# Banksylel/Restrictive-Hierarchical-Semantic-Segmentation

Measured on AMD Instinct MI355X. Metric: train images/sec (620x620, hier-HRNet-W48), higher is better.
Workload: dtype f32 (fp16x2 split on fp16 MFMA, 22-bit operands, fp32 accumulate; exact-fp32 MFMA on the small problems); 1 GPU; HRNet-W48 hierarchical (class_tree_tl.json), 620x620, batch 4 per GPU, train_epoch batch body (fwd L passes, prediction prep + metrics, CE+Dice+consistency, bwd, grad all-reduce, AdamW, metric vectors, one D2H readback of loss+metrics); global_batch=4, parallelism=dp1, launch=launch tape replay, rccl_ranks=1, level_passes=batched (one launch per layer for all L passes)

## Files before the change

restrictive-hierarchical-semantic-segmentation_amd/csrc/bn.hip:

```cpp
#include "elem_common.h"
#include "sp_arith.h"

__device__ __forceinline__ void reduce_chunks16(const double* __restrict__ partial, int nchunks, int C, int c,
                                               double& s0, double& s1, double* red) {
  const int lane = threadIdx.x >> 4;
  double a = 0.0, b = 0.0;
  if (c < C) {
    int k = lane;
    for (; k + 48 < nchunks; k += 64) {
      double t0[4], t1[4];
#pragma unroll
      for (int u = 0; u < 4; ++u) {
        t0[u] = partial[((size_t)(k + 16 * u) * 2 + 0) * C + c];
        t1[u] = partial[((size_t)(k + 16 * u) * 2 + 1) * C + c];
      }
#pragma unroll
      for (int u = 0; u < 4; ++u) {
        a += t0[u];
        b += t1[u];
      }
    }
    for (; k < nchunks; k += 16) {
      a += partial[((size_t)k * 2 + 0) * C + c];
      b += partial[((size_t)k * 2 + 1) * C + c];
    }
  }
  red[threadIdx.x * 2] = a;
  red[threadIdx.x * 2 + 1] = b;
  __syncthreads();
  s0 = 0.0;
  s1 = 0.0;
  if (threadIdx.x < 16)
    for (int l = 0; l < 16; ++l) {
      s0 += red[(l * 16 + threadIdx.x) * 2];
      s1 += red[(l * 16 + threadIdx.x) * 2 + 1];
    }
}

__global__ __launch_bounds__(256) void bn_fold_kernel(const float* __restrict__ w, const float* __restrict__ bias,
                                                      const float* __restrict__ gamma, const float* __restrict__ beta,
                                                      const float* __restrict__ rmean, const float* __restrict__ rvar, float eps,
                                                      int row, float* __restrict__ w_out, float* __restrict__ b_out) {
  const int co = blockIdx.x;
  const float s = (gamma ? gamma[co] : 1.f) / sqrtf(rvar[co] + eps);
  for (int i = threadIdx.x; i < row; i += 256) w_out[(size_t)co * row + i] = w[(size_t)co * row + i] * s;
  if (threadIdx.x == 0) b_out[co] = ((bias ? bias[co] : 0.f) - rmean[co]) * s + (beta ? beta[co] : 0.f);
}

#define BN_MAXG 8
struct BnGroupHdr { int n; int blk_end[BN_MAXG]; };
__device__ __forceinline__ int bn_find(const BnGroupHdr& h, int& local, int& nblk) {
  int g = 0;
  while (g + 1 < h.n && (int)blockIdx.x >= h.blk_end[g]) ++g;
  const int lo = g ? h.blk_end[g - 1] : 0;
  local = blockIdx.x - lo;
  nblk = h.blk_end[g] - lo;
  return g;
}
struct BnFwdG { BnGroupHdr h; hrseg_bn_fwd_t p[BN_MAXG]; };
struct BnBwdG { BnGroupHdr h; hrseg_bn_bwd_t p[BN_MAXG]; };

template <bool MASK>
__device__ __forceinline__ void stats_body(const float* __restrict__ a0, int ld0, const float* __restrict__ zmask,
                                           int ldz, int relu, const float* __restrict__ yy, int ldy,
                                           const float* __restrict__ coef, long npix, int C,
                                           double* __restrict__ partial, int chunk, int nchunks, bool bwd,
                                           double* red, int nseg = 1, const unsigned char* __restrict__ bmask = nullptr) {
  const Lanes L = make_lanes(C);
  const int cps = nchunks / nseg, seg = chunk / cps;
  const long seg_pix = npix / nseg;
  const long per = (seg_pix + cps - 1) / cps;
  const long lo = seg * seg_pix + (long)(chunk - seg * cps) * per;
  const long seg_end = (seg + 1) * seg_pix;
  const long hi = (lo + per < seg_end) ? lo + per : seg_end;
  f32x4 s = {0.f, 0.f, 0.f, 0.f}, s2 = {0.f, 0.f, 0.f, 0.f};
  if (L.active) {
    f32x4 mean = {0.f, 0.f, 0.f, 0.f}, rstd = {1.f, 1.f, 1.f, 1.f}, sc = mean, sh = mean;
    if (bwd) {
      mean = ld4(coef + 4 * L.cq);
      rstd = ld4(coef + C + 4 * L.cq);
      sc = ld4(coef + 2 * C + 4 * L.cq);
      sh = ld4(coef + 3 * C + 4 * L.cq);
// ... 303 lines not shown
          a_dg = f32x4{0.f, 0.f, 0.f, 0.f};
          a_db = f32x4{0.f, 0.f, 0.f, 0.f};
          ++b;
          bnd += hw;
          if (gb) {
            gam = ld4(gb + (size_t)b * 2 * C + 4 * L.cq);
            bet = ld4(gb + (size_t)b * 2 * C + C + 4 * L.cq);
          }
        }
        const f32x4 zc = bn_affine(yv[u], sc, sh);
        f32x4 fv;
#pragma unroll
        for (int j = 0; j < 4; ++j) fv[j] = fmaxf(zc[j], 0.f);
        const f32x4 fm = fv * gam + bet;
        f32x4 uu = {0.f, 0.f, 0.f, 0.f};
#pragma unroll
        for (int c = 0; c < CO; ++c) {
          uu += wq[c] * g[u][c];
          a_dw[c] += fm * g[u][c];
          if (L.cq == 0) a_bias[c] += g[u][c];
        }
        a_dg += fv * uu;
        a_db += uu;
        f32x4 gv = gam * uu;
#pragma unroll
        for (int j = 0; j < 4; ++j) gv[j] = zc[j] > 0.f ? gv[j] : 0.f;
        const f32x4 xh = (yv[u] - mean) * rstd;
        s += gv;
        s2 += gv * xh;
      }
    }
    flush_dgb();
  }
#pragma unroll
  for (int j = 0; j < 4; ++j) {
    red[threadIdx.x * 8 + j] = s[j];
    red[threadIdx.x * 8 + 4 + j] = s2[j];
  }
  __syncthreads();
  for (int c = threadIdx.x; c < C; c += 256) {
    double sa = 0.0, sb = 0.0;
    for (int pl = 0; pl < L.P; ++pl) {
      const int t = pl * L.Q + (c >> 2);
      sa += red[t * 8 + (c & 3)];
      sb += red[t * 8 + 4 + (c & 3)];
    }
    a.partial[((size_t)chunk * 2 + 0) * C + c] = sa;
    a.partial[((size_t)chunk * 2 + 1) * C + c] = sb;
  }
  float* fred = reinterpret_cast<float*>(red);
  float* dw = a.dw[seg];
  float* dbias = a.dbias[seg];
  auto reduce_add = [&](float v, float* dst) {
    __syncthreads();
    fred[threadIdx.x] = v;
    __syncthreads();
    if (L.active && L.pl == 0) {
      float t = 0.f;
      for (int q = 0; q < L.P; ++q) t += fred[q * L.Q + L.cq];
      atomicAdd(dst, t);
    }
  };
#pragma unroll
  for (int j = 0; j < 4; ++j)
#pragma unroll
    for (int c = 0; c < CO; ++c)
      if (c < Cout) reduce_add(a_dw[c][j], dw + c * C + 4 * (L.active ? L.cq : 0) + j);
  if (dbias) {
#pragma unroll
    for (int c = 0; c < CO; ++c)
      if (c < Cout) {
        __syncthreads();
        fred[threadIdx.x] = (L.active && L.cq == 0) ? a_bias[c] : 0.f;
        __syncthreads();
        if (threadIdx.x == 0) {
          float t = 0.f;
          for (int q = 0; q < L.P; ++q) t += fred[q * L.Q];
          atomicAdd(dbias + c, t);
        }
      }
  }
}

template <int CO>
__global__ __launch_bounds__(256) void head_bn_bwd_apply_kernel(hrseg_head_bn_t a) {
  const int C = a.F;
  const Lanes L = make_lanes(C);
  float amax = 0.f;
  if (L.active) {
    const double* totals = a.partial + (size_t)a.nchunks * 2 * C;
    const f32x4 mean = ld4(a.coef + 4 * L.cq), rstd = ld4(a.coef + C + 4 * L.cq), scale = ld4(a.coef + 2 * C + 4 * L.cq);
    const f32x4 shift = ld4(a.coef + 3 * C + 4 * L.cq);
    const long hw = a.hw, seg_pix = (long)a.B * hw;
    const float inv = (float)(1.0 / (double)seg_pix);
    for (int seg = 0; seg < a.nseg; ++seg) {
      f32x4 mg, mgx;
#pragma unroll
      for (int j = 0; j < 4; ++j) {
        mg[j] = (float)(totals[(size_t)seg * 2 * C + 4 * L.cq + j]) * inv;
        mgx[j] = (float)(totals[(size_t)seg * 2 * C + C + 4 * L.cq + j]) * inv;
      }
      const float* __restrict__ gb = a.gb[seg];
      const float* __restrict__ w = a.w[seg];
      const float* __restrict__ dzl = a.dzl[seg];
      const int lddz = a.lddzl[seg], Cout = a.Cout[seg];
      f32x4 wq[CO];
#pragma unroll
      for (int c = 0; c < CO; ++c) wq[c] = (c < Cout) ? ld4(w + c * C + 4 * L.cq) : f32x4{0.f, 0.f, 0.f, 0.f};
      for (int b = 0; b < a.B; ++b) {
        const f32x4 gam = gb ? ld4(gb + (size_t)b * 2 * C + 4 * L.cq) : f32x4{1.f, 1.f, 1.f, 1.f};
        const long r0 = (long)b * hw, r1 = r0 + hw;
        for (long r = r0 + (long)blockIdx.x * L.P + L.pl; r < r1; r += (long)gridDim.x * L.P) {
          const long pix = seg * seg_pix + r;
          const f32x4 yv = ld4(a.y + pix * a.ldy + 4 * L.cq);
          f32x4 uu = {0.f, 0.f, 0.f, 0.f};
#pragma unroll
          for (int c = 0; c < CO; ++c) uu += wq[c] * ((c < Cout) ? dzl[r * lddz + c] : 0.f);
          f32x4 gg = gam * uu;
          const f32x4 zz = bn_affine(yv, scale, shift);
#pragma unroll
          for (int j = 0; j < 4; ++j) gg[j] = zz[j] > 0.f ? gg[j] : 0.f;
          const f32x4 xh = (yv - mean) * rstd;
          const f32x4 dyv = scale * (gg - mg - xh * mgx);
          st4(a.dy + pix * a.lddy + 4 * L.cq, dyv);
#pragma unroll
          for (int j = 0; j < 4; ++j) amax = fmaxf(amax, fabsf(dyv[j]));
        }
      }
    }
  }
  if (a.dy_absmax) {
    __shared__ float wmax[4];
#pragma unroll
    for (int o = 32; o > 0; o >>= 1) amax = fmaxf(amax, __shfl_xor(amax, o, 64));
    if ((threadIdx.x & 63) == 0) wmax[threadIdx.x >> 6] = amax;
    __syncthreads();
    if (threadIdx.x == 0) {
      const float m = fmaxf(fmaxf(wmax[0], wmax[1]), fmaxf(wmax[2], wmax[3]));
      if (m > 0.f) atomicMax(reinterpret_cast<unsigned*>(a.dy_absmax) + (blockIdx.x & 63), __float_as_uint(m));
    }
  }
}

extern "C" int hrseg_bn_fold(const float* w, const float* bias, const float* gamma, const float* beta, const float* running_mean,
                             const float* running_var, float eps, int Cout, int row, float* w_out, float* b_out,
                             hrseg_stream_t stream) {
  HRSEG_CHECK_ARG(w && running_mean && running_var && w_out && b_out && Cout > 0 && row > 0, "hrseg_bn_fold: bad arguments");
  hipLaunchKernelGGL(bn_fold_kernel, dim3(Cout), dim3(256), 0, (hipStream_t)stream, w, bias, gamma, beta, running_mean,
                     running_var, eps, row, w_out, b_out);
  HRSEG_LAUNCH_CHECK("bn_fold");
  return 0;
}

static int check_bn_fwd(const hrseg_bn_fwd_t& p, int training, int phases) {
  if (int e = check_c(p.C, "hrseg_bn_fwd_group")) return e;
  const bool stats = training && (phases & 1), finalize = phases & 2, apply = phases & 4;
  HRSEG_CHECK_ARG(p.coef, "hrseg_bn_fwd_group: bad tensor arguments (coef)");
  HRSEG_CHECK_ARG(!(stats || apply) || (p.y && p.ldy >= p.C && p.ldy % 4 == 0), "hrseg_bn_fwd_group: bad tensor arguments (y, ldy)");
  HRSEG_CHECK_ARG(!(stats || apply || (training && finalize)) || p.npix > 0, "hrseg_bn_fwd_group: bad tensor arguments (npix)");
  HRSEG_CHECK_ARG(!apply || (p.z && p.ldz >= p.C && p.ldz % 4 == 0), "hrseg_bn_fwd_group: bad tensor arguments (the apply phase needs z, ldz)");
  HRSEG_CHECK_ARG(!(stats || (training && finalize)) || (p.partial && p.nchunks > 0), "hrseg_bn_fwd_group: training needs partial/nchunks");
  HRSEG_CHECK_ARG(training || !finalize || (p.running_mean && p.running_var), "hrseg_bn_fwd_group: eval needs running stats");
  return 0;
}

extern "C" int hrseg_bn_fwd_group(int n, const hrseg_bn_fwd_t* probs, int training, hrseg_stream_t stream) {
// ... 26 lines not shown
  } else if (phases & 2) {
    for (int i = 0; i < n; ++i) { end += ceil_div(probs[i].C, 64); g.h.blk_end[i] = end; }
    hipLaunchKernelGGL(bn_eval_coef_group_kernel, dim3(end), dim3(64), 0, st, g);
    HRSEG_LAUNCH_CHECK("bn_eval_coef_group");
  }
  if (phases & 4) {
    end = 0;
    for (int i = 0; i < n; ++i) { end += elem_grid(probs[i].npix, probs[i].C); g.h.blk_end[i] = end; }
    hipLaunchKernelGGL(bn_apply_group_kernel, dim3(end), dim3(256), 0, st, g);
    HRSEG_LAUNCH_CHECK("bn_apply_group");
  }
  return 0;
}

extern "C" int hrseg_bn_bwd_group(int n, const hrseg_bn_bwd_t* probs, int eval_mode, hrseg_stream_t stream) {
  return hrseg_bn_bwd_group_phases(n, probs, eval_mode, 7, stream);
}

extern "C" int hrseg_bn_bwd_group_phases(int n, const hrseg_bn_bwd_t* probs, int eval_mode, int phases, hrseg_stream_t stream) {
  HRSEG_CHECK_ARG(n >= 1 && n <= BN_MAXG && probs, "hrseg_bn_bwd_group: n must be 1..%d", BN_MAXG);
  HRSEG_CHECK_ARG(phases > 0 && phases <= 7, "hrseg_bn_bwd_group_phases: phases is a mask of bits 0..2");
  hipStream_t st = (hipStream_t)stream;
  BnBwdG g;
  g.h.n = n;
  for (int i = 0; i < n; ++i) {
    const hrseg_bn_bwd_t& p = probs[i];
    if (int e = check_c(p.C, "hrseg_bn_bwd_group")) return e;
    HRSEG_CHECK_ARG(p.dz && p.y && p.coef && p.dy && p.partial && p.npix > 0 && p.nchunks > 0,
                    "hrseg_bn_bwd_group: bad arguments");
    HRSEG_CHECK_ARG(p.nseg <= 1 || (p.nchunks % p.nseg == 0 && p.npix % p.nseg == 0),
                    "hrseg_bn_bwd_group: nseg=%d must divide nchunks=%d and npix", p.nseg, p.nchunks);
    g.p[i] = p;
  }
  int end = 0;
  bool masked = false;
  for (int i = 0; i < n; ++i) masked = masked || (probs[i].relu && probs[i].relu_mask);
  if (phases & 1) {
    for (int i = 0; i < n; ++i) { end += probs[i].nchunks; g.h.blk_end[i] = end; }
    if (masked) hipLaunchKernelGGL(bn_bwd_reduce_group_kernel<true>, dim3(end), dim3(256), 0, st, g);
    else hipLaunchKernelGGL(bn_bwd_reduce_group_kernel<false>, dim3(end), dim3(256), 0, st, g);
    HRSEG_LAUNCH_CHECK("bn_bwd_reduce_group");
  }
  if (phases & 2) {
    end = 0;
    for (int i = 0; i < n; ++i) { end += ceil_div(probs[i].C, 16); g.h.blk_end[i] = end; }
    hipLaunchKernelGGL(bn_bwd_finalize_group_kernel, dim3(end), dim3(256), 0, st, g);
    HRSEG_LAUNCH_CHECK("bn_bwd_finalize_group");
  }
  if (phases & 4) {
    end = 0;
    for (int i = 0; i < n; ++i) { end += elem_grid(probs[i].npix, probs[i].C); g.h.blk_end[i] = end; }
    hipLaunchKernelGGL(bn_bwd_apply_group_kernel, dim3(end), dim3(256), 0, st, g, eval_mode);
    HRSEG_LAUNCH_CHECK("bn_bwd_apply_group");
  }
  return 0;
}

static int check_head_bn(const hrseg_head_bn_t* p, const char* who, int seg0, int nsegs) {
  HRSEG_CHECK_ARG(p, "%s: NULL problem", who);
  if (int e = check_c(p->F, who)) return e;
  HRSEG_CHECK_ARG(p->y && p->coef && p->partial && p->B > 0 && p->hw > 0 && p->nseg >= 1 && p->nseg <= HRSEG_HEAD_BN_MAX_SEG &&
                      p->nchunks > 0 && p->nchunks % p->nseg == 0 && p->ldy >= p->F && p->ldy % 4 == 0,
                  "%s: bad arguments (F=%d nseg=%d nchunks=%d ldy=%d)", who, p->F, p->nseg, p->nchunks, p->ldy);
  HRSEG_CHECK_ARG(seg0 >= 0 && nsegs >= 1 && seg0 + nsegs <= p->nseg, "%s: segments [%d, %d) of %d", who, seg0, seg0 + nsegs, p->nseg);
  for (int s = seg0; s < seg0 + nsegs; ++s) {
    HRSEG_CHECK_ARG(p->w[s] && p->dzl[s] && p->Cout[s] > 0 && p->Cout[s] <= 8 && p->lddzl[s] >= p->Cout[s],
                    "%s: segment %d: bad head (Cout=%d lddzl=%d)", who, s, p->Cout[s], p->lddzl[s]);
  }
  return 0;
}

extern "C" int hrseg_head_bn_bwd_reduce(const hrseg_head_bn_t* p, int seg0, int nsegs, hrseg_stream_t stream) {
  if (int e = check_head_bn(p, "hrseg_head_bn_bwd_reduce", seg0, nsegs)) return e;
  if (hrseg_g_deterministic) {
    hrseg_set_error("hrseg_head_bn_bwd_reduce: not offered in deterministic mode (atomic sums); use hrseg_head_bwd + hrseg_bn_bwd_group");
    return HRSEG_ERR_UNSUPPORTED;
  }
  int comax = 0;
  for (int s = seg0; s < seg0 + nsegs; ++s) {
    HRSEG_CHECK_ARG(p->dw[s] && (p->gb[s] == nullptr) == (p->dgb[s] == nullptr), "hrseg_head_bn_bwd_reduce: segment %d: dw is required, dgb goes with gb", s);
    comax = p->Cout[s] > comax ? p->Cout[s] : comax;
  }
  const int cps = p->nchunks / p->nseg;
  if (comax <= 4) hipLaunchKernelGGL(head_bn_bwd_reduce_kernel<4>, dim3(nsegs * cps), dim3(256), 0, (hipStream_t)stream, *p, seg0 * cps);
  else hipLaunchKernelGGL(head_bn_bwd_reduce_kernel<8>, dim3(nsegs * cps), dim3(256), 0, (hipStream_t)stream, *p, seg0 * cps);
  HRSEG_LAUNCH_CHECK("head_bn_bwd_reduce");
  return 0;
}

extern "C" int hrseg_head_bn_bwd_apply(const hrseg_head_bn_t* p, hrseg_stream_t stream) {
  if (int e = check_head_bn(p, "hrseg_head_bn_bwd_apply", 0, p ? p->nseg : 1)) return e;
  HRSEG_CHECK_ARG(p->dy && p->lddy >= p->F && p->lddy % 4 == 0, "hrseg_head_bn_bwd_apply: bad dy (lddy=%d)", p->lddy);
  int comax = 0;
  for (int s = 0; s < p->nseg; ++s) comax = p->Cout[s] > comax ? p->Cout[s] : comax;
  const long npix = (long)p->nseg * p->B * p->hw;
  const int grid = elem_grid(npix, p->F);
  if (comax <= 4) hipLaunchKernelGGL(head_bn_bwd_apply_kernel<4>, dim3(grid), dim3(256), 0, (hipStream_t)stream, *p);
  else hipLaunchKernelGGL(head_bn_bwd_apply_kernel<8>, dim3(grid), dim3(256), 0, (hipStream_t)stream, *p);
  HRSEG_LAUNCH_CHECK("head_bn_bwd_apply");
  return 0;
}
```

restrictive-hierarchical-semantic-segmentation_amd/csrc/head_loss.hip:

```cpp
#include "common.h"

#define MAXC 16

struct Groups {
  int n;
  int parent[MAXC];
  int size[MAXC];
};

static int fill_groups(Groups& g, int ngroups, const int* parent, const int* size, int C, int Cprev, const char* who) {
  HRSEG_CHECK_ARG(ngroups >= 0 && ngroups <= MAXC && (ngroups == 0 || (parent && size)), "%s: bad group table", who);
  g.n = ngroups;
  int tot = 0;
  for (int i = 0; i < ngroups; ++i) {
    HRSEG_CHECK_ARG(parent[i] >= 0 && parent[i] < Cprev && size[i] > 0, "%s: group %d out of range", who, i);
    g.parent[i] = parent[i];
    g.size[i] = size[i];
    tot += size[i];
  }
  HRSEG_CHECK_ARG(tot == C || ngroups == 0, "%s: group sizes sum to %d, level has %d channels", who, tot, C);
  return 0;
}

__global__ __launch_bounds__(256) void gap_partial_kernel(const float* __restrict__ p, double* __restrict__ part,
// ... 240 lines not shown
        for (int c = 0; c < CO; ++c) g[i][c] = (c < Cout) ? dz[r * lddz + c] : 0.f;
      }
#pragma unroll
      for (int i = 0; i < U; ++i) one(fv[i], g[i], dold[i], (size_t)b * hw + pix + (long)i * P);
    }
    for (; pix < hi; pix += P) {
      const size_t r = (size_t)b * hw + pix;
      float g[CO];
#pragma unroll
      for (int c = 0; c < CO; ++c) g[c] = (c < Cout) ? dz[r * lddz + c] : 0.f;
      one(*reinterpret_cast<const f32x4*>(f + r * ldf + 4 * cq), g, racc ? *reinterpret_cast<const f32x4*>(df + r * lddf + 4 * cq) : zero, r);
    }
  }
  auto reduce_add = [&](float v, float* dst) {
    red[threadIdx.x] = v;
    __syncthreads();
    if (active && pl == 0) {
      float s = 0.f;
      for (int q = 0; q < P; ++q) s += red[q * Q + cq];
      atomicAdd(dst, s);
    }
    __syncthreads();
  };
#pragma unroll
  for (int j = 0; j < 4; ++j) {
#pragma unroll
    for (int c = 0; c < CO; ++c)
      if (c < Cout) reduce_add(a_dw[c][j], dw + c * F + 4 * cq + j);
    if (dgb) {
      reduce_add(a_dg[j], dgb + (size_t)b * 2 * F + 4 * cq + j);
      reduce_add(a_db[j], dgb + (size_t)b * 2 * F + F + 4 * cq + j);
    }
  }
  if (dbias) {
#pragma unroll
    for (int c = 0; c < CO; ++c)
      if (c < Cout) {
        red[threadIdx.x] = (active && cq == 0) ? a_bias[c] : 0.f;
        __syncthreads();
        if (threadIdx.x == 0) {
          float s = 0.f;
          for (int q = 0; q < P; ++q) s += red[q * Q];
          atomicAdd(dbias + c, s);
        }
        __syncthreads();
      }
  }
}

__device__ __forceinline__ void src_index_ac(int o, float scale, int in_size, int align, int& i0, int& i1, float& l0,
                                             float& l1) {
  float r;
  if (align) {
    r = scale * (float)o;
  } else {
    r = scale * ((float)o + 0.5f) - 0.5f;
    if (r < 0.f) r = 0.f;
  }
  i0 = (int)r;
  if (i0 > in_size - 1) i0 = in_size - 1;
  i1 = i0 + ((i0 < in_size - 1) ? 1 : 0);
  l1 = r - (float)i0;
  l0 = 1.f - l1;
}
__global__ void logits_up_fwd_kernel(const float* __restrict__ in, int ldin, int B, int Hi, int Wi, int C,
                                     float* __restrict__ out, int Ho, int Wo, float sh, float sw, int align) {
  const long i = (long)blockIdx.x * blockDim.x + threadIdx.x;
  const long hw = (long)Ho * Wo;
  if (i >= B * hw) return;
  const int b = (int)(i / hw);
  const long p = i - b * hw;
  const int oy = (int)(p / Wo), ox = (int)(p - (long)oy * Wo);
  int y0, y1, x0, x1;
  float ly0, ly1, lx0, lx1;
  src_index_ac(oy, sh, Hi, align, y0, y1, ly0, ly1);
  src_index_ac(ox, sw, Wi, align, x0, x1, lx0, lx1);
  const float* base = in + (size_t)b * Hi * Wi * ldin;
  for (int c = 0; c < C; ++c) {
    const float v00 = base[((size_t)y0 * Wi + x0) * ldin + c], v01 = base[((size_t)y0 * Wi + x1) * ldin + c];
    const float v10 = base[((size_t)y1 * Wi + x0) * ldin + c], v11 = base[((size_t)y1 * Wi + x1) * ldin + c];
    out[((size_t)b * C + c) * hw + p] = ly0 * (lx0 * v00 + lx1 * v01) + ly1 * (lx0 * v10 + lx1 * v11);
  }
}
__global__ void logits_up_bwd_kernel(const float* __restrict__ dout, int B, int Hi, int Wi, int C,
                                     float* __restrict__ din, int lddin, int Ho, int Wo, float sh, float sw,
                                     int align) {
  const long i = (long)blockIdx.x * blockDim.x + threadIdx.x;
  if (i >= (long)B * Hi * Wi) return;
  const int b = (int)(i / ((long)Hi * Wi));
  const int rem = (int)(i - (long)b * Hi * Wi);
  const int iy = rem / Wi, ix = rem - iy * Wi;
  const long hw = (long)Ho * Wo;
  const float ish = sh > 0.f ? 1.f / sh : 0.f, isw = sw > 0.f ? 1.f / sw : 0.f;
  const float hf = align ? 0.f : 0.5f;
  int oy_lo = 0, oy_hi = Ho - 1, ox_lo = 0, ox_hi = Wo - 1;
  if (sh > 0.f) {
    oy_lo = max(0, (int)floorf(((float)iy - 1.f + hf) * ish - hf) - 1);
    oy_hi = min(Ho - 1, (int)ceilf(((float)iy + 1.f + hf) * ish - hf) + 1);
  }
  if (sw > 0.f) {
    ox_lo = max(0, (int)floorf(((float)ix - 1.f + hf) * isw - hf) - 1);
    ox_hi = min(Wo - 1, (int)ceilf(((float)ix + 1.f + hf) * isw - hf) + 1);
  }
  float s[MAXC];
#pragma unroll
  for (int c = 0; c < MAXC; ++c) s[c] = 0.f;
  for (int oy = oy_lo; oy <= oy_hi; ++oy) {
    int y0, y1;
    float ly0, ly1;
    src_index_ac(oy, sh, Hi, align, y0, y1, ly0, ly1);
    const float wy = (y0 == iy ? ly0 : 0.f) + (y1 == iy ? ly1 : 0.f);
    if (wy == 0.f) continue;
    for (int ox = ox_lo; ox <= ox_hi; ++ox) {
      int x0, x1;
      float lx0, lx1;
      src_index_ac(ox, sw, Wi, align, x0, x1, lx0, lx1);
      const float wx = (x0 == ix ? lx0 : 0.f) + (x1 == ix ? lx1 : 0.f);
      if (wx == 0.f) continue;
      const float wgt = wy * wx;
#pragma unroll
      for (int c = 0; c < MAXC; ++c)
        if (c < C) s[c] = fmaf(wgt, dout[((size_t)b * C + c) * hw + (size_t)oy * Wo + ox], s[c]);
    }
  }
#pragma unroll
  for (int c = 0; c < MAXC; ++c)
    if (c < C) din[i * lddin + c] = s[c];
}

__global__ void sigmoid_fwd_kernel(const float* __restrict__ z, float* __restrict__ p, long n) {
  const long i = (long)blockIdx.x * blockDim.x + threadIdx.x;
  if (i < n) p[i] = 1.f / (1.f + expf(-z[i]));
}
__global__ void sigmoid_bwd_kernel(const float* __restrict__ dp, long sb, long sc, long si,
                                   const float* __restrict__ z, float* __restrict__ dz, int acc, int C, long hw,
                                   long n) {
  const long i = (long)blockIdx.x * blockDim.x + threadIdx.x;
  if (i >= n) return;
  const long bc = i / hw, pix = i - bc * hw;
  const long b = bc / C, c = bc - b * C;
  const float p = 1.f / (1.f + expf(-z[i]));
  const float g = dp[b * sb + c * sc + pix * si] * p * (1.f - p);
  dz[i] = acc ? dz[i] + g : g;
}

#define EPS_GATE 1e-6f
__global__ void compose_fwd_kernel(const float* __restrict__ z, const float* __restrict__ pprev,
                                   float* __restrict__ p, int C, int Cprev, long hw, long n, Groups g) {
  const long i = (long)blockIdx.x * blockDim.x + threadIdx.x;
  if (i >= n) return;
  const long b = i / hw, pix = i - b * hw;
  const float* zb = z + (size_t)b * C * hw + pix;
  float* pb = p + (size_t)b * C * hw + pix;
  int start = 0;
  for (int gi = 0; gi < g.n; ++gi) {
    const int sz = g.size[gi];
    const float pp = pprev[((size_t)b * Cprev + g.parent[gi]) * hw + pix];
    const float lg = logf(pp + EPS_GATE);
    float m = -INFINITY;
    for (int c = 0; c < sz; ++c) m = fmaxf(m, zb[(size_t)(start + c) * hw] + lg);
    float s = 0.f;
    for (int c = 0; c < sz; ++c) s += expf(zb[(size_t)(start + c) * hw] + lg - m);
    const float inv = 1.f / s;
    for (int c = 0; c < sz; ++c) pb[(size_t)(start + c) * hw] = pp * (expf(zb[(size_t)(start + c) * hw] + lg - m) * inv);
    start += sz;
  }
}
__global__ void compose_bwd_kernel(const float* __restrict__ dp, long sb, long sc, long si,
                                   const float* __restrict__ z, const float* __restrict__ pprev,
                                   float* __restrict__ dz, int dz_acc, float* __restrict__ dpprev, int dpp_acc,
                                   int C, int Cprev, long hw, long n, Groups g) {
  const long i = (long)blockIdx.x * blockDim.x + threadIdx.x;
  if (i >= n) return;
  const long b = i / hw, pix = i - b * hw;
  const float* zb = z + (size_t)b * C * hw + pix;
  float dpar[MAXC];
#pragma unroll
  for (int c = 0; c < MAXC; ++c) dpar[c] = 0.f;
  int start = 0;
  for (int gi = 0; gi < g.n; ++gi) {
    const int sz = g.size[gi];
    const float pp = pprev[((size_t)b * Cprev + g.parent[gi]) * hw + pix];
    const float lg = logf(pp + EPS_GATE);
    float m = -INFINITY;
    for (int c = 0; c < sz; ++c) m = fmaxf(m, zb[(size_t)(start + c) * hw] + lg);
    float s = 0.f;
    for (int c = 0; c < sz; ++c) s += expf(zb[(size_t)(start + c) * hw] + lg - m);
    const float inv = 1.f / s;
    float dot = 0.f, dpp = 0.f;
    for (int c = 0; c < sz; ++c) {
      const float q = expf(zb[(size_t)(start + c) * hw] + lg - m) * inv;
      const float d = dp[b * sb + (start + c) * sc + pix * si];
      dot += q * d * pp;
      dpp += d * q;
    }
    float sum_ds = 0.f;
    for (int c = 0; c < sz; ++c) {
      const float q = expf(zb[(size_t)(start + c) * hw] + lg - m) * inv;
      const float d = dp[b * sb + (start + c) * sc + pix * si];
      const float ds = q * (d * pp - dot);
      sum_ds += ds;
      if (dz) {
        float* o = dz + ((size_t)b * C + start + c) * hw + pix;
        *o = dz_acc ? *o + ds : ds;
      }
    }
    dpp += sum_ds / (pp + EPS_GATE);
#pragma unroll
    for (int c = 0; c < MAXC; ++c)
      if (c == g.parent[gi]) dpar[c] += dpp;
// ... 385 lines not shown
  const size_t smem = (size_t)(co * F + co) * sizeof(float);
  const int lp = (F / 4 <= 16) ? 16 : 64;
  long blocks = (hw + (256 / lp) - 1) / (256 / lp);
  const long cap = (2048 + B - 1) / B < 64 ? 64 : (2048 + B - 1) / B;
  if (blocks > cap) blocks = cap;
  dim3 grid((int)blocks, B);
#define HF(LP_, CO_)                                                                                                              \
  do {                                                                                                                            \
    if (coef) hipLaunchKernelGGL((head_fwd_kernel<LP_, CO_, true>), grid, dim3(256), smem, st, f, ldf, coef, gb, w, bias, z, ldz, \
                                 hw, F, Cout);                                                                                    \
    else hipLaunchKernelGGL((head_fwd_kernel<LP_, CO_, false>), grid, dim3(256), smem, st, f, ldf, coef, gb, w, bias, z, ldz, hw, \
                            F, Cout);                                                                                             \
  } while (0)
  if (lp == 16 && co == 4) HF(16, 4);
  else if (lp == 16) HF(16, 8);
  else if (co == 4) HF(64, 4);
  else HF(64, 8);
#undef HF
  HRSEG_LAUNCH_CHECK(who);
  return 0;
}

extern "C" int hrseg_head_fwd(const float* f, int ldf, const float* gb, const float* w, const float* bias, float* z,
                              int ldz, int B, long hw, int F, int Cout, hrseg_stream_t stream) {
  return head_fwd_launch("hrseg_head_fwd", f, ldf, nullptr, gb, w, bias, z, ldz, B, hw, F, Cout, stream);
}

extern "C" int hrseg_head_bn_fwd(const float* y, int ldy, const float* coef, const float* gb, const float* w, const float* bias,
                                 float* z, int ldz, int B, long hw, int F, int Cout, hrseg_stream_t stream) {
  HRSEG_CHECK_ARG(coef, "hrseg_head_bn_fwd: coef is required (hrseg_head_fwd reads a normalised tensor)");
  return head_fwd_launch("hrseg_head_bn_fwd", y, ldy, coef, gb, w, bias, z, ldz, B, hw, F, Cout, stream);
}

extern "C" int hrseg_head_bwd(const float* f, int ldf, const float* gb, const float* w, const float* dz, int lddz,
                              float* df, int lddf, int df_accumulate, float* dw, float* dbias, float* dgb, int B,
                              long hw, int F, int Cout, hrseg_stream_t stream) {
  HRSEG_CHECK_ARG(f && w && dz && dw && B > 0 && hw > 0 && F > 0 && F % 4 == 0 && F <= 1024 && Cout > 0 &&
                      Cout <= 8 && (gb == nullptr) == (dgb == nullptr),
                  "hrseg_head_bwd: bad arguments (F=%d Cout=%d)", F, Cout);
  HRSEG_CHECK_ARG(ldf >= F && ldf % 4 == 0 && lddz >= Cout && (df == nullptr || (lddf >= F && lddf % 4 == 0)),
                  "hrseg_head_bwd: bad row strides (ldf=%d lddz=%d lddf=%d for F=%d Cout=%d)", ldf, lddz, lddf, F, Cout);
  hipStream_t st = (hipStream_t)stream;
  long chunks = 2048 / B;
  if (chunks < 1) chunks = 1;
  long ppb = (hw + chunks - 1) / chunks;
  if (ppb < 64) ppb = 64;
  const int nlaunch = hrseg_g_deterministic ? B : 1;
  if (hrseg_g_deterministic) ppb = hw;
  dim3 grid(ceil_div(hw, ppb), hrseg_g_deterministic ? 1 : B);
  for (int b0 = 0; b0 < nlaunch; ++b0) {
    if (Cout <= 4)
      hipLaunchKernelGGL((head_bwd_kernel<4>), grid, dim3(256), 0, st, f, ldf, gb, w, dz, lddz, df, lddf, df_accumulate,
                         dw, dbias, dgb, hw, F, Cout, ppb, b0);
    else
      hipLaunchKernelGGL((head_bwd_kernel<8>), grid, dim3(256), 0, st, f, ldf, gb, w, dz, lddz, df, lddf, df_accumulate,
                         dw, dbias, dgb, hw, F, Cout, ppb, b0);
  }
  HRSEG_LAUNCH_CHECK("head_bwd");
  return 0;
}

static float up_scale(int in_size, int out_size, int align) {
  if (align) return out_size > 1 ? (float)(in_size - 1) / (float)(out_size - 1) : 0.f;
  return (float)in_size / (float)out_size;
}

extern "C" int hrseg_logits_up_fwd(const float* in, int ldin, int B, int Hi, int Wi, int C, float* out, int Ho, int Wo,
                                   int align_corners, hrseg_stream_t stream) {
  HRSEG_CHECK_ARG(in && out && B > 0 && Hi > 0 && Wi > 0 && Ho > 0 && Wo > 0 && C > 0 && C <= MAXC && ldin >= C,
                  "hrseg_logits_up_fwd: bad arguments");
  const long n = (long)B * Ho * Wo;
  hipLaunchKernelGGL(logits_up_fwd_kernel, dim3(ceil_div(n, 256)), dim3(256), 0, (hipStream_t)stream, in, ldin, B, Hi,
                     Wi, C, out, Ho, Wo, up_scale(Hi, Ho, align_corners), up_scale(Wi, Wo, align_corners),
                     align_corners);
  HRSEG_LAUNCH_CHECK("logits_up_fwd");
  return 0;
}

extern "C" int hrseg_logits_up_bwd(const float* dout, int B, int Hi, int Wi, int C, float* din, int lddin, int Ho,
                                   int Wo, int align_corners, hrseg_stream_t stream) {
  HRSEG_CHECK_ARG(dout && din && B > 0 && Hi > 0 && Wi > 0 && Ho > 0 && Wo > 0 && C > 0 && C <= MAXC && lddin >= C,
                  "hrseg_logits_up_bwd: bad arguments");
  const long n = (long)B * Hi * Wi;
  hipLaunchKernelGGL(logits_up_bwd_kernel, dim3(ceil_div(n, 128)), dim3(128), 0, (hipStream_t)stream, dout, B, Hi, Wi,
                     C, din, lddin, Ho, Wo, up_scale(Hi, Ho, align_corners), up_scale(Wi, Wo, align_corners),
                     align_corners);
  HRSEG_LAUNCH_CHECK("logits_up_bwd");
  return 0;
}

extern "C" int hrseg_sigmoid_fwd(const float* z, float* p, long n, hrseg_stream_t stream) {
  HRSEG_CHECK_ARG(z && p && n > 0, "hrseg_sigmoid_fwd: bad arguments");
  hipLaunchKernelGGL(sigmoid_fwd_kernel, dim3(ceil_div(n, 256)), dim3(256), 0, (hipStream_t)stream, z, p, n);
  HRSEG_LAUNCH_CHECK("sigmoid_fwd");
  return 0;
}

extern "C" int hrseg_sigmoid_bwd(const float* dp, long sb, long sc, long si, const float* z, float* dz, int accumulate,
                                 int B, int C, long hw, hrseg_stream_t stream) {
  HRSEG_CHECK_ARG(dp && z && dz && B > 0 && C > 0 && hw > 0, "hrseg_sigmoid_bwd: bad arguments");
  const long n = (long)B * C * hw;
  hipLaunchKernelGGL(sigmoid_bwd_kernel, dim3(ceil_div(n, 256)), dim3(256), 0, (hipStream_t)stream, dp, sb, sc, si, z,
                     dz, accumulate, C, hw, n);
  HRSEG_LAUNCH_CHECK("sigmoid_bwd");
  return 0;
}

extern "C" int hrseg_compose_fwd(const float* z, const float* pprev, float* p, int B, int C, int Cprev, long hw,
                                 int ngroups, const int* group_parent, const int* group_size, hrseg_stream_t stream) {
  HRSEG_CHECK_ARG(z && pprev && p && B > 0 && C > 0 && C <= MAXC && Cprev > 0 && Cprev <= MAXC && hw > 0 && ngroups > 0,
                  "hrseg_compose_fwd: bad arguments");
  Groups g;
  if (int e = fill_groups(g, ngroups, group_parent, group_size, C, Cprev, "hrseg_compose_fwd")) return e;
  const long n = (long)B * hw;
  hipLaunchKernelGGL(compose_fwd_kernel, dim3(ceil_div(n, 256)), dim3(256), 0, (hipStream_t)stream, z, pprev, p, C,
                     Cprev, hw, n, g);
  HRSEG_LAUNCH_CHECK("compose_fwd");
  return 0;
}

extern "C" int hrseg_compose_bwd(const float* dp, long sb, long sc, long si, const float* z, const float* pprev,
                                 float* dz, int dz_accumulate, float* dpprev, int dpprev_accumulate, int B, int C,
                                 int Cprev, long hw, int ngroups, const int* group_parent, const int* group_size,
                                 hrseg_stream_t stream) {
  HRSEG_CHECK_ARG(dp && z && pprev && B > 0 && C > 0 && C <= MAXC && Cprev > 0 && Cprev <= MAXC && hw > 0 && ngroups > 0,
                  "hrseg_compose_bwd: bad arguments");
  Groups g;
  if (int e = fill_groups(g, ngroups, group_parent, group_size, C, Cprev, "hrseg_compose_bwd")) return e;
  const long n = (long)B * hw;
  hipLaunchKernelGGL(compose_bwd_kernel, dim3(ceil_div(n, 256)), dim3(256), 0, (hipStream_t)stream, dp, sb, sc, si, z,
                     pprev, dz, dz_accumulate, dpprev, dpprev_accumulate, C, Cprev, hw, n, g);
  HRSEG_LAUNCH_CHECK("compose_bwd");
  return 0;
}

extern "C" int hrseg_loss_partials(const float* z, const float* t, double* partial, int B, int C, long hw,
                                   hrseg_stream_t stream) {
  HRSEG_CHECK_ARG(z && t && partial && B > 0 && C > 0 && C <= MAXC && hw > 0, "hrseg_loss_partials: bad arguments (C=%d)", C);
  hipStream_t st = (hipStream_t)stream;
  hipLaunchKernelGGL(zero_f64_kernel, dim3(1), dim3(256), 0, st, partial, B * C * 5);
  long chunks = hrseg_g_deterministic ? 1 : 1024 / B;
  if (chunks < 1) chunks = 1;
  long ppb = (hw + chunks - 1) / chunks;
  if (ppb < 256) ppb = 256;
  dim3 grid(ceil_div(hw, ppb), B);
  if (C <= 4) hipLaunchKernelGGL((loss_partials_kernel<4>), grid, dim3(256), 0, st, z, t, partial, C, hw, ppb);
  else if (C <= 8) hipLaunchKernelGGL((loss_partials_kernel<8>), grid, dim3(256), 0, st, z, t, partial, C, hw, ppb);
  else hipLaunchKernelGGL((loss_partials_kernel<16>), grid, dim3(256), 0, st, z, t, partial, C, hw, ppb);
  HRSEG_LAUNCH_CHECK("loss_partials");
  return 0;
}

extern "C" int hrseg_loss_finalize(const double* partial, const float* w, int B, int C, float* out, float* coef,
                                   hrseg_stream_t stream) {
  HRSEG_CHECK_ARG(partial && w && out && coef && B > 0 && C > 0, "hrseg_loss_finalize: bad arguments");
  hipLaunchKernelGGL(loss_finalize_kernel, dim3(1), dim3(64), 0, (hipStream_t)stream, partial, w, B, C, out, coef);
  HRSEG_LAUNCH_CHECK("loss_finalize");
  return 0;
}

extern "C" int hrseg_loss_bwd(const float* z, const float* t, const float* coef, const float* g, float* dz,
                              int accumulate, int B, int C, long hw, hrseg_stream_t stream) {
  HRSEG_CHECK_ARG(z && t && coef && g && dz && B > 0 && C > 0 && C <= MAXC && hw > 0, "hrseg_loss_bwd: bad arguments");
  hipStream_t st = (hipStream_t)stream;
  dim3 grid(ceil_div(hw, 256), B);
  if (C <= 4) hipLaunchKernelGGL((loss_bwd_kernel<4>), grid, dim3(256), 0, st, z, t, coef, g, dz, accumulate, C, hw);
  else if (C <= 8) hipLaunchKernelGGL((loss_bwd_kernel<8>), grid, dim3(256), 0, st, z, t, coef, g, dz, accumulate, C, hw);
// ... 205 lines not shown
```

Baseline: 92.43 images/s.

## Add warp-specialized LDS ring for head BN backward reduce; parallelize upsample bwd over channels

```diff
diff --git a/restrictive-hierarchical-semantic-segmentation_amd/csrc/bn.hip b/restrictive-hierarchical-semantic-segmentation_amd/csrc/bn.hip
--- a/restrictive-hierarchical-semantic-segmentation_amd/csrc/bn.hip
+++ b/restrictive-hierarchical-semantic-segmentation_amd/csrc/bn.hip
@@ -1,3 +1,4 @@
+#include <type_traits>
 #include "elem_common.h"
 #include "sp_arith.h"
 
@@ -467,6 +468,210 @@
   }
 }
 
+#define HEAD_RING_ROWS 16
+static size_t head_ring_lds_bytes(int F) { return (size_t)2 * HEAD_RING_ROWS * (F + 8) * sizeof(float); }
+template <int CO>
+__global__ __launch_bounds__(512) void head_bn_bwd_reduce_ring_kernel(hrseg_head_bn_t a, int chunk0) {
+  extern __shared__ __attribute__((aligned(16))) float ring[];
+  constexpr int R = HEAD_RING_ROWS;
+  const int C = a.F, Q = C >> 2;
+  float* const ybuf = ring;
+  float* const gbuf = ring + (size_t)2 * R * C;
+  const bool loader = __builtin_amdgcn_readfirstlane((int)threadIdx.x) >= 256;
+  const int cq = threadIdx.x & 255;
+  const bool active = cq < Q;
+  const int chunk = chunk0 + blockIdx.x;
+  const int cps = a.nchunks / a.nseg, seg = chunk / cps;
+  const long hw = a.hw, seg_pix = (long)a.B * hw;
+  const long per = (seg_pix + cps - 1) / cps;
+  const long seg_base = seg * seg_pix;
+  const long lo = seg_base + (long)(chunk - seg * cps) * per;
+  const long seg_end = seg_base + seg_pix;
+  const long hi = (lo + per < seg_end) ? lo + per : seg_end;
+  const int nst = lo < hi ? (int)(((hi - lo + R - 1) / R + 1) & ~1L) : 0;
+  if (blockIdx.x == 0 && threadIdx.x < 64 && a.dy_absmax) a.dy_absmax[threadIdx.x] = 0.f;
+  const float* __restrict__ gb = a.gb[seg];
+  const float* __restrict__ w = a.w[seg];
+  const float* __restrict__ dzl = a.dzl[seg];
+  const int lddz = a.lddzl[seg], Cout = a.Cout[seg];
+  float* dgb = a.dgb[seg];
+  auto stage_barrier = [&]() {
+    asm volatile("s_waitcnt lgkmcnt(0)" ::: "memory");
+    __builtin_amdgcn_s_barrier();
+  };
+  if (loader) {
+    if (nst > 0) {
+      const int lcq = active ? cq : Q - 1, gr = cq & (R - 1);
+      f32x4 va[R], vb[R];
+      float ga[CO], gv[CO];
+      auto issue = [&](f32x4 (&v)[R], float (&g)[CO], int st) {
+        const long p0 = lo + (long)st * R;
+        asm volatile("" ::: "memory");
+#pragma unroll
+        for (int r = 0; r < R; ++r) {
+          const long pix = (p0 + r < hi) ? p0 + r : hi - 1;
+          v[r] = ld4(a.y + pix * a.ldy + 4 * lcq);
+        }
+        const long gp = (p0 + gr < hi) ? p0 + gr : hi - 1;
+#pragma unroll
+        for (int c = 0; c < CO; ++c) g[c] = dzl[(gp - seg_base) * lddz + (c < Cout ? c : Cout - 1)];
+        asm volatile("" ::: "memory");
+      };
+      auto write = [&](const f32x4 (&v)[R], const float (&g)[CO], int st) {
+        float* ys = ybuf + (size_t)(st & 1) * R * C + 4 * lcq;
+#pragma unroll
+        for (int r = 0; r < R; ++r) st4(ys + r * C, v[r]);
+        float* gs = gbuf + ((st & 1) * R + gr) * 8;
+#pragma unroll
+        for (int c = 0; c < CO; ++c) gs[c] = (c < Cout) ? g[c] : 0.f;
+      };
+      issue(va, ga, 0);
+      issue(vb, gv, 1);
+      write(va, ga, 0);
+      issue(va, ga, 2);
+      stage_barrier();
+      for (int t = 0; t < nst; t += 2) {
+        write(vb, gv, t + 1);
+        issue(vb, gv, t + 3);
+        stage_barrier();
+        write(va, ga, t + 2);
+        issue(va, ga, t + 4);
+        stage_barrier();
+      }
+    }
+    return;
+  }
+  f32x4 s = {0.f, 0.f, 0.f, 0.f}, s2 = {0.f, 0.f, 0.f, 0.f};
+  f32x4 a_dw[CO], a_dg = {0.f, 0.f, 0.f, 0.f}, a_db = {0.f, 0.f, 0.f, 0.f};
+  float a_bias[CO];
+#pragma unroll
+  for (int c = 0; c < CO; ++c) {
+    a_dw[c] = f32x4{0.f, 0.f, 0.f, 0.f};
+    a_bias[c] = 0.f;
+  }
+  const int bias_tid = Q <= 192 ? 192 : 0;
+  const bool bias_wave = (__builtin_amdgcn_readfirstlane((int)threadIdx.x) >> 6) == (bias_tid >> 6);
+  float* dbias = a.dbias[seg];
+  if (nst > 0) {
+    const int ccq = active ? cq : 0;
+    const f32x4 mean = ld4(a.coef + 4 * ccq), rstd = ld4(a.coef + C + 4 * ccq);
+    const f32x4 sc = ld4(a.coef + 2 * C + 4 * ccq), sh = ld4(a.coef + 3 * C + 4 * ccq);
+    f32x4 wq[CO];
+#pragma unroll
+    for (int c = 0; c < CO; ++c) wq[c] = (c < Cout) ? ld4(w + c * C + 4 * ccq) : f32x4{0.f, 0.f, 0.f, 0.f};
+    long b = (lo - seg_base) / hw;
+    long bnd = seg_base + (b + 1) * hw;
+    f32x4 gam = {1.f, 1.f, 1.f, 1.f}, bet = {0.f, 0.f, 0.f, 0.f};
+    if (gb) {
+      gam = ld4(gb + (size_t)b * 2 * C + 4 * ccq);
+      bet = ld4(gb + (size_t)b * 2 * C + C + 4 * ccq);
+    }
+    auto flush_dgb = [&]() {
+      if (dgb && active) {
+#pragma unroll
+        for (int j = 0; j < 4; ++j) {
+          atomicAdd(dgb + (size_t)b * 2 * C + 4 * cq + j, a_dg[j]);
+          atomicAdd(dgb + (size_t)b * 2 * C + C + 4 * cq + j, a_db[j]);
+        }
+      }
+    };
+    auto one = [&](auto with_bias, const float* ys, const float* gs) {
+      const f32x4 yv = ld4(ys);
+      float g[CO];
+      const f32x4 g0 = ld4(gs);
+#pragma unroll
+      for (int c = 0; c < (CO < 4 ? CO : 4); ++c) g[c] = g0[c];
+      if (CO > 4) {
+        const f32x4 g1 = ld4(gs + 4);
+#pragma unroll
+        for (int c = 4; c < CO; ++c) g[c] = g1[c - 4];
+      }
+      const f32x4 zc = bn_affine(yv, sc, sh);
+      f32x4 fv;
+#pragma unroll
+      for (int j = 0; j < 4; ++j) fv[j] = fmaxf(zc[j], 0.f);
+      const f32x4 fm = fv * gam + bet;
+      f32x4 uu = {0.f, 0.f, 0.f, 0.f};
+#pragma unroll
+      for (int c = 0; c < CO; ++c) {
+        uu += wq[c] * g[c];
+        a_dw[c] += fm * g[c];
+        if (decltype(with_bias)::value) a_bias[c] += g[c];
+      }
+      a_dg += fv * uu;
+      a_db += uu;
+      f32x4 gv = gam * uu;
+#pragma unroll
+      for (int j = 0; j < 4; ++j) gv[j] = zc[j] > 0.f ? gv[j] : 0.f;
+      const f32x4 xh = (yv - mean) * rstd;
+      s += gv;
+      s2 += gv * xh;
+    };
+    auto stages = [&](auto with_bias) {
+    stage_barrier();
+    for (int t = 0; t < nst; ++t) {
+      const float* ys = ybuf + (size_t)(t & 1) * R * C + 4 * ccq;
+      const float* gs = gbuf + (t & 1) * R * 8;
+      const long p0 = lo + (long)t * R;
+      if (p0 + R <= hi && p0 + R <= bnd) {
+        constexpr int UR = CO <= 4 ? R : 4;
+#pragma unroll 1
+        for (int r0 = 0; r0 < R; r0 += UR)
+#pragma unroll
+          for (int r = r0; r < r0 + UR; ++r) one(with_bias, ys + r * C, gs + r * 8);
+      } else {
+        for (int r = 0; r < R && p0 + r < hi; ++r) {
+          while (p0 + r >= bnd) {
+            flush_dgb();
+            a_dg = f32x4{0.f, 0.f, 0.f, 0.f};
+            a_db = f32x4{0.f, 0.f, 0.f, 0.f};
+            ++b;
+            bnd += hw;
+            if (gb) {
+              gam = ld4(gb + (size_t)b * 2 * C + 4 * ccq);
+              bet = ld4(gb + (size_t)b * 2 * C + C + 4 * ccq);
+            }
+          }
+          one(with_bias, ys + r * C, gs + r * 8);
+        }
+      }
+      stage_barrier();
+    }
+    };
+    if (bias_wave) stages(std::true_type());
+    else stages(std::false_type());
+    flush_dgb();
+  }
+  if (dbias && (int)threadIdx.x == bias_tid) {
+#pragma unroll
+    for (int c = 0; c < CO; ++c)
+      if (c < Cout) {
+        float t = 0.f;
+        t += a_bias[c];
+        atomicAdd(dbias + c, t);
+      }
+  }
+  if (!active) return;
+#pragma unroll
+  for (int j = 0; j < 4; ++j) {
+    double sa = 0.0, sb = 0.0;
+    sa += (double)s[j];
+    sb += (double)s2[j];
+    a.partial[((size_t)chunk * 2 + 0) * C + 4 * cq + j] = sa;
+    a.partial[((size_t)chunk * 2 + 1) * C + 4 * cq + j] = sb;
+  }
+  float* dw = a.dw[seg];
+#pragma unroll
+  for (int j = 0; j < 4; ++j)
+#pragma unroll
+    for (int c = 0; c < CO; ++c)
+      if (c < Cout) {
+        float t = 0.f;
+        t += a_dw[c][j];
+        atomicAdd(dw + c * C + 4 * cq + j, t);
+      }
+}
+
 template <int CO>
 __global__ __launch_bounds__(256) void head_bn_bwd_apply_kernel(hrseg_head_bn_t a) {
   const int C = a.F;
@@ -659,7 +864,22 @@
     comax = p->Cout[s] > comax ? p->Cout[s] : comax;
   }
   const int cps = p->nchunks / p->nseg;
-  if (comax <= 4) hipLaunchKernelGGL(head_bn_bwd_reduce_kernel<4>, dim3(nsegs * cps), dim3(256), 0, (hipStream_t)stream, *p, seg0 * cps);
+  if (p->F / 4 > 128) {
+    const size_t lds = head_ring_lds_bytes(p->F);
+    static bool raised = false;
+    if (!raised) {
+      const int most = (int)head_ring_lds_bytes(1024);
+      const hipError_t e4 = hipFuncSetAttribute(reinterpret_cast<const void*>(&head_bn_bwd_reduce_ring_kernel<4>), hipFuncAttributeMaxDynamicSharedMemorySize, most);
+      const hipError_t e8 = hipFuncSetAttribute(reinterpret_cast<const void*>(&head_bn_bwd_reduce_ring_kernel<8>), hipFuncAttributeMaxDynamicSharedMemorySize, most);
+      if (e4 != hipSuccess || e8 != hipSuccess) {
+        hrseg_set_error("hrseg_head_bn_bwd_reduce: %d bytes of LDS refused: %s", most, hipGetErrorString(e4 != hipSuccess ? e4 : e8));
+        return HRSEG_ERR_LAUNCH;
+      }
+      raised = true;
+    }
+    if (comax <= 4) hipLaunchKernelGGL(head_bn_bwd_reduce_ring_kernel<4>, dim3(nsegs * cps), dim3(512), lds, (hipStream_t)stream, *p, seg0 * cps);
+    else hipLaunchKernelGGL(head_bn_bwd_reduce_ring_kernel<8>, dim3(nsegs * cps), dim3(512), lds, (hipStream_t)stream, *p, seg0 * cps);
+  } else if (comax <= 4) hipLaunchKernelGGL(head_bn_bwd_reduce_kernel<4>, dim3(nsegs * cps), dim3(256), 0, (hipStream_t)stream, *p, seg0 * cps);
   else hipLaunchKernelGGL(head_bn_bwd_reduce_kernel<8>, dim3(nsegs * cps), dim3(256), 0, (hipStream_t)stream, *p, seg0 * cps);
   HRSEG_LAUNCH_CHECK("head_bn_bwd_reduce");
   return 0;
diff --git a/restrictive-hierarchical-semantic-segmentation_amd/csrc/head_loss.hip b/restrictive-hierarchical-semantic-segmentation_amd/csrc/head_loss.hip
--- a/restrictive-hierarchical-semantic-segmentation_amd/csrc/head_loss.hip
+++ b/restrictive-hierarchical-semantic-segmentation_amd/csrc/head_loss.hip
@@ -346,13 +346,26 @@
     out[((size_t)b * C + c) * hw + p] = ly0 * (lx0 * v00 + lx1 * v01) + ly1 * (lx0 * v10 + lx1 * v11);
   }
 }
+__device__ __forceinline__ float tap_weight(int o, float scale, int in_size, int align, int i) {
+  int i0, i1;
+  float l0, l1;
+  src_index_ac(o, scale, in_size, align, i0, i1, l0, l1);
+  return (i0 == i ? l0 : 0.f) + (i1 == i ? l1 : 0.f);
+}
+__device__ __forceinline__ void tap_range(int& lo, int& hi, float scale, int in_size, int align, int i) {
+  while (lo <= hi && tap_weight(lo, scale, in_size, align, i) == 0.f) ++lo;
+  while (hi > lo && tap_weight(hi, scale, in_size, align, i) == 0.f) --hi;
+}
 __global__ void logits_up_bwd_kernel(const float* __restrict__ dout, int B, int Hi, int Wi, int C,
                                      float* __restrict__ din, int lddin, int Ho, int Wo, float sh, float sw,
                                      int align) {
   const long i = (long)blockIdx.x * blockDim.x + threadIdx.x;
-  if (i >= (long)B * Hi * Wi) return;
-  const int b = (int)(i / ((long)Hi * Wi));
-  const int rem = (int)(i - (long)b * Hi * Wi);
+  const long npix = (long)B * Hi * Wi;
+  if (i >= npix * C) return;
+  const int c = (int)(i / npix);
+  const long pix = i - (long)c * npix;
+  const int b = (int)(pix / ((long)Hi * Wi));
+  const int rem = (int)(pix - (long)b * Hi * Wi);
   const int iy = rem / Wi, ix = rem - iy * Wi;
   const long hw = (long)Ho * Wo;
   const float ish = sh > 0.f ? 1.f / sh : 0.f, isw = sw > 0.f ? 1.f / sw : 0.f;
@@ -366,30 +379,21 @@
     ox_lo = max(0, (int)floorf(((float)ix - 1.f + hf) * isw - hf) - 1);
     ox_hi = min(Wo - 1, (int)ceilf(((float)ix + 1.f + hf) * isw - hf) + 1);
   }
-  float s[MAXC];
-#pragma unroll
-  for (int c = 0; c < MAXC; ++c) s[c] = 0.f;
+  tap_range(oy_lo, oy_hi, sh, Hi, align, iy);
+  tap_range(ox_lo, ox_hi, sw, Wi, align, ix);
+  const float* __restrict__ plane = dout + ((size_t)b * C + c) * hw;
+  float s = 0.f;
   for (int oy = oy_lo; oy <= oy_hi; ++oy) {
-    int y0, y1;
-    float ly0, ly1;
-    src_index_ac(oy, sh, Hi, align, y0, y1, ly0, ly1);
-    const float wy = (y0 == iy ? ly0 : 0.f) + (y1 == iy ? ly1 : 0.f);
+    const float wy = tap_weight(oy, sh, Hi, align, iy);
     if (wy == 0.f) continue;
     for (int ox = ox_lo; ox <= ox_hi; ++ox) {
-      int x0, x1;
-      float lx0, lx1;
-      src_index_ac(ox, sw, Wi, align, x0, x1, lx0, lx1);
-      const float wx = (x0 == ix ? lx0 : 0.f) + (x1 == ix ? lx1 : 0.f);
+      const float wx = tap_weight(ox, sw, Wi, align, ix);
       if (wx == 0.f) continue;
       const float wgt = wy * wx;
-#pragma unroll
-      for (int c = 0; c < MAXC; ++c)
-        if (c < C) s[c] = fmaf(wgt, dout[((size_t)b * C + c) * hw + (size_t)oy * Wo + ox], s[c]);
-    }
-  }
-#pragma unroll
-  for (int c = 0; c < MAXC; ++c)
-    if (c < C) din[i * lddin + c] = s[c];
+      s = fmaf(wgt, plane[(size_t)oy * Wo + ox], s);
+    }
+  }
+  din[pix * lddin + c] = s;
 }
 
 __global__ void sigmoid_fwd_kernel(const float* __restrict__ z, float* __restrict__ p, long n) {
@@ -941,7 +945,7 @@
   HRSEG_CHECK_ARG(dout && din && B > 0 && Hi > 0 && Wi > 0 && Ho > 0 && Wo > 0 && C > 0 && C <= MAXC && lddin >= C,
                   "hrseg_logits_up_bwd: bad arguments");
   const long n = (long)B * Hi * Wi;
-  hipLaunchKernelGGL(logits_up_bwd_kernel, dim3(ceil_div(n, 128)), dim3(128), 0, (hipStream_t)stream, dout, B, Hi, Wi,
+  hipLaunchKernelGGL(logits_up_bwd_kernel, dim3(ceil_div(n * C, 128)), dim3(128), 0, (hipStream_t)stream, dout, B, Hi, Wi,
                      C, din, lddin, Ho, Wo, up_scale(Hi, Ho, align_corners), up_scale(Wi, Wo, align_corners),
                      align_corners);
   HRSEG_LAUNCH_CHECK("logits_up_bwd");
```

Result: faster. 93.98 images/s (median of 6 runs) (+1.7%).
